# facebookresearch/unbiased-teacher-v2

Measured on AMD Instinct MI355X. Metric: images/sec/node (labeled+unlabeled) UTv2 step, R50-FPN 1333x800, higher is better.
Workload: dtype f16

## Files before the change

include/utv2.h:

```cpp
#ifndef UTV2_H
#define UTV2_H
#include <stdint.h>
#ifdef __cplusplus
extern "C" {
#endif

typedef struct ihipStream_t* utv2_stream_t;

int utv2_conv2d_nhwc_fwd(const float* x, const float* w, float* y, const float* scale, const float* bias,
                         const float* residual, int N, int H, int W, int C, int K, int KH, int KW, int stride, int pad,
                         int in_dil, int OH, int OW, int relu, int accumulate, int Kred, utv2_stream_t stream);
int utv2_conv2d_stem_fwd(const float* x, const float* w, void* y, int y_dtype, const float* scale, const float* bias, int N,
                         int H, int W, int K, int KH, int KW, int stride, int pad, int OH, int OW, int relu, int Kred,
                         utv2_stream_t stream);
int utv2_conv2d_wgrad_splits(int N, int OH, int OW, int K, int Kred);
int64_t utv2_conv2d_wgrad_workspace_floats(int N, int OH, int OW, int K, int Kred);
int utv2_conv2d_nhwc_wgrad(const float* x, const float* dy, float* dw, float* ws, int N, int H, int W, int C, int K,
                           int KH, int KW, int stride, int pad, int OH, int OW, int accumulate, utv2_stream_t stream);
int utv2_colsum(const float* g, float* db, float* ws, int M, int C, int accumulate, utv2_stream_t stream);
int utv2_weight_flip_transpose(const float* w, float* wt, int K, int KH, int KW, int C, utv2_stream_t stream);

int utv2_conv2d_ml_fwd(const float* x, const float* w, float* y, const float* scale, const float* bias,
                       const float* residual, int nlev, const int* H_host, const int* W_host, int N, int C, int K, int KH,
                       int KW, int pad, int relu, int accumulate, utv2_stream_t stream);
// ... 167 lines not shown

int utv2_nms_mpad(int M);
int64_t utv2_nms_workspace_bytes(int N, int M);
int utv2_nms_batched(const float* boxes, const float* scores, const int* cls, const unsigned char* valid, int N, int M,
                     float iou_thr, int class_aware, int post_topk, int max_out, int* keep, int* keep_count, void* ws,
                     utv2_stream_t stream);
int utv2_box_iou(const float* a, const float* b, int A, int B, float* out, utv2_stream_t stream);

int utv2_match_boxes(const float* boxes, int64_t box_img_stride, int N, int P, const float* gt_boxes,
                     const unsigned char* gt_valid, int G, float* max_iou, int* arg, unsigned* gt_max_bits,
                     utv2_stream_t stream);
int utv2_match_lowq(const float* boxes, int64_t box_img_stride, int N, int P, const float* gt_boxes,
                    const unsigned char* gt_valid, int G, const unsigned* gt_max_bits, unsigned char* lowq,
                    utv2_stream_t stream);
int utv2_roi_align_fwd(int num_levels, int min_level, const void* const* feats_host, const int* H_host,
                       const int* W_host, const float* scales_host, const float* rois, const int* roi_batch,
                       const unsigned char* roi_valid, int R, int C, int PH, int PW, void* out, int dtype,
                       utv2_stream_t stream);
int utv2_roi_align_bwd(int num_levels, int min_level, float* const* dfeats_host, const int* H_host, const int* W_host,
                       const float* scales_host, const float* rois, const int* roi_batch, const unsigned char* roi_valid,
                       int R, int C, int PH, int PW, const void* dy, int dtype, utv2_stream_t stream);
int utv2_roi_align_bwd_tiled(int num_levels, int min_level, void* const* dfeats_host, const int* H_host, const int* W_host,
                             const float* scales_host, const float* rois, const unsigned char* roi_valid, int N, int rois_per_image,
                             int C, int PH, int PW, const void* dy, int dy_dtype, int out_dtype, utv2_stream_t stream);
int utv2_rpn_rank_keys(const float* head, int num_levels, const int* hw_host, int N, int A, int ch, int64_t* keys, utv2_stream_t stream);
int utv2_rpn_decode(const int64_t* top, int maxk, const float* head, const float* anchors, const float* image_hw, int num_levels,
                    const int* hw_host, const int* k_host, int N, int A, int ch, const float* weights_host, float scale_clamp,
                    float min_size, float* boxes, float* scores, int* lvls, unsigned char* keep, utv2_stream_t stream);
int utv2_nms_pack(const int* kidx, const int* cnt, const float* boxes, const float* scores, int N, int M, int D, float* oboxes, float* oscores,
                  unsigned char* ovalid, utv2_stream_t stream);
int utv2_roi_infer_keys(const float* probs, const float* deltas, const float* prop, const unsigned char* valid, const float* whwh, int N, int P,
                        int K, float wx, float wy, float scale_clamp, float thr, float* boxes, int64_t* keys, utv2_stream_t stream);
int utv2_roi_infer_gather(const int64_t* top, const float* boxes, int N, int P, int K, int k, float thr, float* sc, int64_t* rows, int* cls,
                          float* cb, unsigned char* valid, utv2_stream_t stream);
int utv2_roi_infer_pack(const int* kidx, const int* cnt, const float* cb, const float* sc, const int* cls, const int64_t* rows, const float* stdl,
                        int N, int P, int k, int D, float* oboxes, float* oscores, int* ocls, float* ostd, int64_t* orows, unsigned char* ovalid,
                        utv2_stream_t stream);
int utv2_rpn_loss_fwd(const float* obj, const float* deltas, int head, int num_levels, const int* hw_host, int N, int A, int ch, int R,
                      const float* anchors, const int64_t* pos_idx, const unsigned char* pos_valid, int npos, const int64_t* neg_idx,
                      const unsigned char* neg_valid, int nneg, const int* matched, const unsigned char* has_gt, const float* gt_boxes,
                      const float* gt_scores, int G, const float* weights_host, float* sums, float* gobj, float* gdl, utv2_stream_t stream);
int utv2_rpn_loss_bwd(const float* gobj, const float* gdl, const float* gout_cls, const float* gout_loc, int head, int num_levels,
                      const int* hw_host, int N, int A, int ch, int R, const int64_t* pos_idx, const unsigned char* pos_valid, int npos,
                      const int64_t* neg_idx, const unsigned char* neg_valid, int nneg, float* grad_obj, float* grad_deltas,
                      utv2_stream_t stream);
int utv2_rpn_loss_fwd_range(const float* obj, const float* deltas, int head, int num_levels, const int* hw_host, int N, int batch, int img0,
                            int A, int ch, int R, const float* anchors, const int64_t* pos_idx, const unsigned char* pos_valid, int npos,
                            const int64_t* neg_idx, const unsigned char* neg_valid, int nneg, const int* matched,
                            const unsigned char* has_gt, const float* gt_boxes, const float* gt_scores, int G, const float* weights_host,
                            float* sums, float* gobj, float* gdl, utv2_stream_t stream);
int utv2_rpn_loss_bwd_range(const float* gobj, const float* gdl, const float* gout_cls, const float* gout_loc, int head, int num_levels,
                            const int* hw_host, int N, int batch, int img0, int A, int ch, int R, const int64_t* pos_idx,
                            const unsigned char* pos_valid, int npos, const int64_t* neg_idx, const unsigned char* neg_valid, int nneg,
                            float* grad_obj, float* grad_deltas, utv2_stream_t stream);
int utv2_rpn_sample_keys(const float* max_iou, const unsigned char* lowq, const unsigned char* gt_valid, int G, const float* keys, int N,
                         int R, float lo, float hi, int64_t* out, utv2_stream_t stream);
int utv2_rpn_sample_unpack(const int64_t* top, int k, int N, int npos_max, int nneg_max, const unsigned char* gt_valid, int G,
                           int64_t* pos_idx, unsigned char* pos_valid, int64_t* neg_idx, unsigned char* neg_valid, unsigned char* has_gt,
                           utv2_stream_t stream);
int utv2_roi_sample(const float* boxes, const unsigned char* valid, const float* max_iou, const int* argmax, const float* keys, int N, int P,
                    const float* gt_boxes, const int* gt_classes, const unsigned char* gt_valid, const float* gt_scores, const float* gt_std,
                    int G, float iou_thr, int num_classes, int batch, int nfg_max, float* out_boxes, int64_t* out_classes,
                    float* out_gt_boxes, unsigned char* out_valid, int64_t* out_idx, float* out_conf, float* out_std, utv2_stream_t stream);
int utv2_roi_box_loss(const float* deltas, const float* stdl, int64_t ld, const int64_t* cls, const float* prop, const float* gtb,
                      const float* gstd, int R, int num_classes, int mode, float wx, float wy, float scale_clamp, float ts_better,
                      float t_cert, float* sum, float* gdeltas, float* gstd_out, utv2_stream_t stream);
int utv2_softmax_focal_fwd(const float* logits, const int* target, int R, int C, float gamma, float* loss_sum, float* ws,
                           utv2_stream_t stream);
int utv2_softmax_focal_bwd(const float* logits, const int* target, int R, int C, float gamma, const float* coef,
                           float* dlogits, utv2_stream_t stream);
int utv2_rcnn_loss_combine(const float* rpn_sup, const float* rpn_uns, const float* focal_sup, const float* focal_uns, const float* box_sup,
                           const float* box_uns, const int* tgt_sup, int n_sup, const int* tgt_uns, int n_uns, float rpn_norm_sup,
                           float rpn_norm_uns, float w_rpn_cls, float w_rpn_loc, float w_box, const float* wt_host, float* rec, float* coef,
                           utv2_stream_t stream);

int utv2_stem_pool_fwd_bf16(const void* xpad16, const void* w16s, void* y, const float* scale, const float* shift, int N, int H, int W,
                            int K, utv2_stream_t stream);

int utv2_bottleneck_supported(int C, int MID, int has_shortcut);
int utv2_bottleneck_fwd_bf16(const void* x, void* y, const void* w1, const void* w2, const void* w3, const void* wsc, const float* s1,
                             const float* b1, const float* s2, const float* b2, const float* s3, const float* b3, const float* ssc,
                             const float* bsc, int N, int H, int W, int C, int MID, utv2_stream_t stream);

int64_t utv2_aug_resize_workspace_bytes(int H, int W, int OH, int OW);
int utv2_aug_resize_bilinear_u8(const unsigned char* src, int H, int W, unsigned char* dst, int OH, int OW, int flip, void* ws,
                                utv2_stream_t stream);
int utv2_aug_gray_mean_u8(const unsigned char* img, int64_t npix, void* sum_ws, int* mean_out, utv2_stream_t stream);
int utv2_aug_blend_u8(unsigned char* img, int64_t npix, int mode, float alpha, const int* mean, utv2_stream_t stream);
int utv2_aug_hue_u8(unsigned char* img, int64_t npix, int shift, utv2_stream_t stream);
int utv2_aug_grayscale_u8(unsigned char* img, int64_t npix, utv2_stream_t stream);
int utv2_aug_box_blur_u8(const unsigned char* src, unsigned char* dst, int H, int W, int vertical, int radius, int ww, int fw,
                         utv2_stream_t stream);
int utv2_aug_erase_u8(unsigned char* img, int H, int W, int i, int j, int h, int w, const float* noise, utv2_stream_t stream);
int utv2_aug_hwc_to_chw_u8(const unsigned char* src, unsigned char* dst, int64_t npix, utv2_stream_t stream);

int utv2_coco_pair_keys(const float* scores, const int* cls, const long long* off, int N, int K, long long* keys, utv2_stream_t stream);
int utv2_coco_seg_offsets(const long long* keys, int64_t n, int64_t nseg, long long* off, utv2_stream_t stream);
int utv2_coco_rank_keys(const long long* key1, const long long* pair_off, int64_t D, int K, int max_dets, long long* key2,
                        unsigned char* rank, utv2_stream_t stream);
int64_t utv2_coco_eval_workspace_bytes(int64_t D, int K);
int utv2_coco_match(const float* dbox, const long long* dperm, const long long* dpair_off, const double* gbox, const unsigned char* gcrowd,
                    const double* garea, const long long* gperm, const long long* gpair_off, int N, int K, int64_t D, int max_dets,
                    int max_gt, const double* iou_thrs_host, const double* area_rng_host, void* ws, utv2_stream_t stream);
int utv2_coco_accumulate(const long long* perm2, const long long* cat_off, const unsigned char* rank, int K, int64_t D,
                         const double* rec_thrs_host, const void* ws, double* precision, double* recall, utv2_stream_t stream);

int utv2_gconv3x3_supported(int C, int G);
int utv2_gconv3x3_fwd(const void* x, const void* w, int op_dtype, void* y, int y_dtype, const float* scale, const float* shift, int N,
                      int H, int W, int C, int G, int stride, int OH, int OW, int relu, utv2_stream_t stream);
int utv2_gconv3x3_dgrad(const void* dy, const void* w, int op_dtype, void* dx, int dx_dtype, const float* scale, const void* mask,
                        const void* residual, int N, int H, int W, int C, int G, int stride, int OH, int OW, utv2_stream_t stream);
int utv2_gconv3x3_wgrad_splits(int N, int OH, int OW, int C, int G);
int64_t utv2_gconv3x3_wgrad_workspace_floats(int N, int OH, int OW, int C, int G);
int utv2_gconv3x3_wgrad(const void* x, const void* dy, int op_dtype, float* dw, float* ws, const float* scale, int N, int H, int W,
                        int C, int G, int stride, int OH, int OW, int accumulate, utv2_stream_t stream);

#ifdef __cplusplus
}
#endif
#endif
```

unbiased-teacher-v2_amd/ubteacher/hip.py:

```python
import ctypes
import os

import torch

_HERE = os.path.dirname(os.path.abspath(__file__))
_LIB_DIR = os.environ.get("UTV2_LIB_DIR") or os.path.join(os.path.dirname(_HERE), "lib")
LIB_PATH = os.path.join(_LIB_DIR, "libutv2_hip.so")
LIB_PATHS = {"bf16": LIB_PATH, "fp16": os.path.join(_LIB_DIR, "libutv2_hip_f16.so")}
H16 = ["bf16"]


_H16_DT = [torch.bfloat16]


def set_h16(kind):
    assert kind in LIB_PATHS
    H16[0] = kind
    _H16_DT[0] = torch.bfloat16 if kind == "bf16" else torch.float16


def h16_dtype():
    return _H16_DT[0]

_lib = None

c_p = ctypes.c_void_p
c_i = ctypes.c_int
c_i64 = ctypes.c_int64
c_f = ctypes.c_float

HEADER_PATH = os.path.join(os.path.dirname(os.path.dirname(_HERE)), "include", "utv2.h")


def _parse_header(path):
    import re

    txt = open(path).read()
    txt = re.sub(r"/\*.*?\*/", "", txt, flags=re.S)
    sigs = {}
    for m in re.finditer(r"\b(int64_t|int)\s+(utv2_\w+)\s*\(([^;{]*?)\)\s*;", txt, flags=re.S):
        ret, name, args = m.group(1), m.group(2), m.group(3)
        argt = []
        for a in [x.strip() for x in args.replace("\n", " ").split(",") if x.strip()]:
            if "*" in a or "utv2_stream_t" in a:
                argt.append(c_p)
            elif a.startswith("int64_t"):
                argt.append(c_i64)
            elif a.startswith("double"):
                argt.append(ctypes.c_double)
            elif a.startswith("float"):
                argt.append(c_f)
            elif a.startswith("int"):
                argt.append(c_i)
            elif a == "void":
                pass
            else:
                raise RuntimeError("utv2.h: cannot map argument %r of %s" % (a, name))
        sigs[name] = (c_i64 if ret == "int64_t" else c_i, argt)
    return sigs


_SIGS = _parse_header(HEADER_PATH)
_PLAIN = {"utv2_aug_resize_workspace_bytes", "utv2_topk_rows_workspace_bytes", "utv2_groupnorm_seg_workspace_floats", "utv2_groupnorm_seg_chunks", "utv2_conv2d_wgrad_bf16_splits", "utv2_conv2d_wgrad_bf16_workspace_floats", "utv2_conv2d_bf16_supported", "utv2_conv2d_wgrad_splits", "utv2_conv2d_wgrad_workspace_floats", "utv2_groupnorm_workspace_floats",
          "utv2_nms_mpad", "utv2_nms_workspace_bytes", "utv2_bottleneck_supported", "utv2_wgrad_fold_table_bytes", "utv2_wgrad_fold_pending",
          "utv2_coco_eval_workspace_bytes", "utv2_gconv3x3_supported", "utv2_gconv3x3_wgrad_splits",
          "utv2_gconv3x3_wgrad_workspace_floats"}


_libs = {}


def load(kind=None):
    kind = kind or H16[0]
    lib = _libs.get(kind)
    if lib is not None:
        return lib
    path = LIB_PATHS[kind]
    if not os.path.exists(path):
        raise RuntimeError(
            "HIP extension %s is missing - run `python __graft_entry__.py` (hipcc, gfx950)" % path
        )
    lib = ctypes.CDLL(path)
    for name, (res, args) in _SIGS.items():
        fn = getattr(lib, name)
        fn.restype = res
        fn.argtypes = args
    _libs[kind] = lib
    return lib


def symbols():
    return sorted(_SIGS)


_RAW_STREAM = getattr(torch._C, "_cuda_getCurrentRawStream", None)
_GET_DEVICE = getattr(torch._C, "_cuda_getDevice", None)


def _stream():
    if _RAW_STREAM is not None and _GET_DEVICE is not None:
        return _RAW_STREAM(_GET_DEVICE())
    return torch.cuda.current_stream().cuda_stream


def _p(t):
    if t is None:
        return None
    assert t.is_cuda and t.is_contiguous(), "HIP ops need contiguous CUDA tensors"
    return t.data_ptr()


def _dt(t):
    d = t.dtype
    if d == torch.float32:
        return 0
    if d == _H16_DT[0]:
        return 1
    raise TypeError("activation tensors are fp32 or %s (the selected library's 16-bit type), got %s" % (h16_dtype(), t.dtype))


def _same_dt(*ts):
    ts = [t for t in ts if t is not None]
    assert all(t.dtype == ts[0].dtype for t in ts), [t.dtype for t in ts]
    return _dt(ts[0])


def _p_any(t):
    return c_p(t.data_ptr())


def _check(rc, name):
    if rc != 0:
        raise RuntimeError("%s failed with code %d" % (name, rc))


_FN = {}


def call(name, *args):
    fn = _FN.get((H16[0], name))
    if fn is None:
        fn = _FN[(H16[0], name)] = getattr(load(), name)
    rc = fn(*args)
    if rc != 0:
        raise RuntimeError("%s failed with code %d" % (name, rc))


# ... 747 lines not shown


def f32_to_bf16(src, dst16):
    call("utv2_f32_to_bf16", _p(src), _p(dst16), src.numel(), _stream())


def weight_flip_transpose_bf16(w, K, kh, kw, C, scale=None):
    wt = torch.empty((C, kh * kw * K), dtype=h16_dtype(), device=w.device)
    call("utv2_weight_flip_transpose_bf16", _p(w), _p(wt), _p(scale), K, kh, kw, C, _stream())
    return wt


def _act_dtype(x, out_dtype):
    return out_dtype if out_dtype is not None else x.dtype


def pad_cols_bf16(src2d, cpad):
    rows, c = src2d.shape
    out = torch.empty((rows, cpad), dtype=h16_dtype(), device=src2d.device)
    call("utv2_pad_cols_bf16", _p(src2d), _dt(src2d), _p(out), rows, c, cpad, _stream())
    return out


def weight_flip_transpose_bf16_batched(arena, scales, bank, table, nlayers):
    call("utv2_weight_flip_transpose_bf16_batched", _p(arena), c_p(scales.data_ptr()) if scales is not None else c_p(0), _p(bank),
         _p(table), int(nlayers), _stream())


def relu_bits_buffer(shape, device):
    assert shape[-1] % 8 == 0
    return torch.empty(tuple(shape[:-1]) + (shape[-1] // 8,), dtype=torch.uint8, device=device)


def _bits_ok(bits, shape):
    n = 1
    for d in shape:
        n *= int(d)
    assert bits.dtype == torch.uint8 and bits.is_contiguous() and bits.numel() * 8 == n, "bit plane of another tensor"
    return bits


def conv2d_fwd_bf16(x, w16, scale=None, bias=None, residual=None, stride=1, pad=0, relu=False, kh=1, kw=1, out=None,
                    in_dil=1, out_hw=None, accumulate=False, out_dtype=None, mask=None, post_mask=None, relu_bits=None):
    N, H, W, C = x.shape
    K = w16.shape[0]
    assert w16.dtype == h16_dtype() and C % 8 == 0
    if out_hw is None:
        OH, OW = conv_out_size(H, kh, stride, pad), conv_out_size(W, kw, stride, pad)
    else:
        OH, OW = out_hw
    if out is None:
        out = torch.empty((N, OH, OW, K), dtype=_act_dtype(x, out_dtype), device=x.device)
    ri = None
    if _CONV_ROWINFO and kh * kw > 1 and in_dil == 1 and x.dtype == h16_dtype() and C % 32 == 0 and kh * kw <= 16 and W < 32768:
        ri = rowinfo_nhwc(N, H, W, OH, OW, stride, pad, kh, kw, x.device)
    if relu_bits is not None:
        assert out.dtype == h16_dtype()
        call("utv2_conv2d_nhwc_fwd_bf16_bits", _p(x), _dt(x), _p(w16), _p(out), _same_dt(out, residual, mask, post_mask), _p(scale), _p(bias),
             _p(residual), _p(mask), _p(post_mask), N, H, W, C, K, kh, kw, stride, pad, in_dil, OH, OW, int(relu), int(accumulate), _p(ri),
             _p(_bits_ok(relu_bits, out.shape)), c_p(0), c_p(0), _stream())
        return out
    call("utv2_conv2d_nhwc_fwd_bf16_ri", _p(x), _dt(x), _p(w16), _p(out), _same_dt(out, residual, mask, post_mask), _p(scale), _p(bias),
         _p(residual), _p(mask), _p(post_mask), N, H, W, C, K, kh, kw, stride, pad, in_dil, OH, OW, int(relu), int(accumulate), _p(ri), _stream())
    return out


def bottleneck_fwd_bf16(x, w1, w2, w3, s1, b1, s2, b2, s3, b3, wsc=None, ssc=None, bsc=None, out=None):
    N, H, W, C = x.shape
    MID, K = w1.shape[0], w3.shape[0]
    assert x.dtype == h16_dtype() and w1.dtype == w2.dtype == w3.dtype == h16_dtype() and K == 256
    assert tuple(w1.shape) == (MID, C) and tuple(w2.shape) == (MID, 9 * MID) and tuple(w3.shape) == (K, MID)
    assert wsc is None or (tuple(wsc.shape) == (K, C) and wsc.dtype == h16_dtype())
    if out is None:
        out = torch.empty((N, H, W, K), dtype=x.dtype, device=x.device)
    call("utv2_bottleneck_fwd_bf16", _p(x), _p(out), _p(w1), _p(w2), _p(w3), _p(wsc), _p(s1), _p(b1), _p(s2), _p(b2), _p(s3), _p(b3),
         _p(ssc), _p(bsc), N, H, W, C, MID, _stream())
    return out


def bottleneck_supported(C, MID, has_shortcut):
    return bool(load().utv2_bottleneck_supported(C, MID, int(has_shortcut)))


def conv2d_dgrad_bf16(dy, wt16, in_shape, stride, pad, kh, kw, out=None, out_dtype=None, mask=None, residual=None, post_mask=None,
                      mask_bits=None, post_mask_bits=None):
    N, H, W, C = in_shape
    _, OH, OW, K = dy.shape
    if out is None:
        out = torch.empty((N, H, W, C), dtype=_act_dtype(dy, out_dtype), device=dy.device)
    ri = None
    if _CONV_ROWINFO and kh * kw > 1 and stride == 1 and dy.dtype == h16_dtype() and K % 32 == 0 and kh * kw <= 16 and OW < 32768:
        ri = rowinfo_nhwc(N, OH, OW, H, W, 1, kh - 1 - pad, kh, kw, dy.device)
    if mask_bits is not None or post_mask_bits is not None:
        assert out.dtype == h16_dtype() and (mask is None or mask_bits is None) and (post_mask is None or post_mask_bits is None)
        call("utv2_conv2d_nhwc_fwd_bf16_bits", _p(dy), _dt(dy), _p(wt16), _p(out), _same_dt(out, residual, mask, post_mask), c_p(0), c_p(0),
             _p(residual), _p(mask), _p(post_mask), N, OH, OW, K, C, kh, kw, 1, kh - 1 - pad, stride, H, W, 0, 0, _p(ri), c_p(0),
             _p(_bits_ok(mask_bits, out.shape)) if mask_bits is not None else c_p(0),
             _p(_bits_ok(post_mask_bits, out.shape)) if post_mask_bits is not None else c_p(0), _stream())
        return out
    call("utv2_conv2d_nhwc_fwd_bf16_ri", _p(dy), _dt(dy), _p(wt16), _p(out), _same_dt(out, residual, mask, post_mask), c_p(0), c_p(0),
         _p(residual), _p(mask), _p(post_mask), N, OH, OW, K, C, kh, kw, 1, kh - 1 - pad, stride, H, W, 0, 0, _p(ri), _stream())
    return out


def _rows_ptr(t):
    assert t.is_cuda and t.dim() == 2 and t.stride(1) == 1 and t.stride(0) >= t.shape[1], "row-major matrix (or a column slice of one) expected"
    return c_p(t.data_ptr()), int(t.stride(0))


def gnb_eligible(x2d, w16, k, pad, groups):
    C = x2d.shape[1] // groups
    K = w16.shape[0]
    return (x2d.dtype == h16_dtype() and C % 64 == 0 and k * k * C >= 1024 and K % groups == 0 and (K // groups) % 128 == 0
            and x2d.stride(1) == 1 and x2d.stride(0) % 8 == 0 and x2d.shape[0] * x2d.stride(0) < (1 << 31))


def gnb_part_buffer(P, K, device):
    return torch.empty(((P + 63) // 64, K, 2), dtype=torch.float32, device=device)


def conv2d_ml_fwd_bf16(x2d, w16, level_hw, N, scale=None, bias=None, residual=None, k=3, pad=1, relu=False, out=None,
                       out_dtype=None, groups=1, gn_part=None, gnb=None):
    P = x2d.shape[0]
    C = x2d.shape[1] // groups
    K = w16.shape[0]
    assert w16.shape[1] == k * k * C, (tuple(w16.shape), k, C)
    if out is None:
        out = torch.empty((P, K), dtype=_act_dtype(x2d, out_dtype), device=x2d.device)
    H = _iarr([h for h, _ in level_hw]); W = _iarr([w_ for _, w_ in level_hw])
    xp, xpitch = _rows_ptr(x2d)
    yp, ypitch = _rows_ptr(out)
    if gnb is not None:
        bits, gx, part = gnb
        assert (scale is None and bias is None and residual is None and not relu and gn_part is None and out.dtype == h16_dtype()
                and ypitch == K and gx.dtype == h16_dtype() and gx.is_contiguous() and tuple(gx.shape) == (P, K)
                and bits.numel() * bits.element_size() * 8 == P * K and tuple(part.shape) == ((P + 63) // 64, K, 2))
        ri = rowinfo_ml(N, level_hw, pad, k, x2d.device) if (_CONV_ROWINFO and k > 1) else None
        call("utv2_conv2d_ml_fwd_bf16_gnb", xp, xpitch, _p(w16), yp, len(level_hw), ctypes.cast(H, c_p), ctypes.cast(W, c_p), N, C, K, k, k,
             pad, int(groups), _p(ri), _p(bits), _p(gx), _p(part), _stream())
        return out
    ri = None
    if (_CONV_ROWINFO and k > 1 and x2d.dtype == h16_dtype() and C % 32 == 0 and K % 4 == 0 and xpitch % 8 == 0 and ypitch % 8 == 0
            and (groups == 1 or (K // groups) % 128 == 0) and P * xpitch < (1 << 31)):
        ri = rowinfo_ml(N, level_hw, pad, k, x2d.device)
    if groups == 1 and xpitch == C and ypitch == K and gn_part is None and ri is None:
        call("utv2_conv2d_ml_fwd_bf16", xp, _dt(x2d), _p(w16), yp, _same_dt(out, residual), _p(scale), _p(bias), _p(residual),
             len(level_hw), ctypes.cast(H, c_p), ctypes.cast(W, c_p), N, C, K, k, k, pad, int(relu), 0, _stream())
    else:
        assert residual is None or (residual.stride(0) == ypitch and residual.stride(1) == 1)
        call("utv2_conv2d_ml_fwd_bf16_g", xp, _dt(x2d), xpitch, _p(w16), yp, _same_dt(out, residual), ypitch, _p(scale), _p(bias),
             c_p(residual.data_ptr()) if residual is not None else c_p(0), len(level_hw), ctypes.cast(H, c_p), ctypes.cast(W, c_p), N, C, K,
             k, k, pad, int(relu), 0, int(groups), _p(gn_part), _p(ri), _stream())
    return out


def gn_part_buffer(P, K, device):
    return torch.empty(((P + 31) // 32, K // 8, 2), dtype=torch.float32, device=device)


def groupnorm_relu_seg_fwd_p32(x2d, seg_rows, gamma, beta, part32, G, eps=1e-5, relu=True, relu_bits=None):
    rows, C = x2d.shape
    assert sum(seg_rows) == rows and x2d.dtype == h16_dtype() and C == 8 * G
    y = torch.empty_like(x2d)
    S = len(seg_rows)
    mean = torch.empty((S, G), dtype=torch.float32, device=x2d.device)
    rstd = torch.empty((S, G), dtype=torch.float32, device=x2d.device)
# ... 346 lines not shown
```

unbiased-teacher-v2_amd/ubteacher/ops.py:

```python
import os

import torch

from . import hip

_HOOKS = {}
PRECISION = ["fp32"]


def set_precision(p):
    assert p in ("fp32", "bf16", "fp16")
    PRECISION[0] = p
    hip.set_h16("fp16" if p == "fp16" else "bf16")


def amp():
    return PRECISION[0] != "fp32"


def act_dtype():
    return hip.h16_dtype() if amp() else torch.float32


_VERSION = [0]
# ... 595 lines not shown
        _wgrad_launch(lambda: hip.gconv3x3_wgrad(x4, g4, layer.w.g, layer.groups, layer.stride, scale=layer.bn.scale, accumulate=True),
                      x4, g4, key=layer)
        return
    n_, h_, w_, _ = x4.shape
    ri = hip.rowinfo_nhwc(n_, h_, w_, g4.shape[1], g4.shape[2], layer.stride, layer.pad, layer.k, layer.k, x4.device)
    _wgrad_launch(lambda: hip.conv2d_wgrad_bf16(x4, g4.reshape(-1, layer.cout), layer.w.g, ri, layer.cin, layer.k, layer.k, accumulate=True,
                                                rowscale=layer.bn.scale), x4, g4, key=layer)


def _dgrad16(layer, g4, in_shape, mask=None, residual=None, post_mask=None, mask_bits=None, post_mask_bits=None):
    if mask_bits is not None:
        mask = None
    if post_mask_bits is not None:
        post_mask = None
    if layer.gconv:
        assert post_mask is None and post_mask_bits is None and mask_bits is None
        return hip.gconv3x3_dgrad(g4, layer.gconv_weight(), layer.groups, layer.stride, tuple(in_shape), scale=layer.bn.scale, mask=mask,
                                  residual=residual, out_dtype=hip.h16_dtype())
    BITS_STATS["reads"] += (mask_bits is not None) + (post_mask_bits is not None)
    return hip.conv2d_dgrad_bf16(g4, layer.wt16(layer.bn.scale), tuple(in_shape), layer.stride, layer.pad, layer.k, layer.k,
                                 out_dtype=hip.h16_dtype(), mask=mask, residual=residual, post_mask=post_mask, mask_bits=mask_bits,
                                 post_mask_bits=post_mask_bits)


class GradHandoff:
    _live = []

    def __init__(self):
        self.grad = None
        self.closed = False
        if len(GradHandoff._live) >= 64:
            del GradHandoff._live[:32]
        GradHandoff._live.append(self)

    def park(self, g):
        if self.closed or self.grad is not None:
            return False
        self.grad = g
        return True

    def take(self):
        self.closed = True
        g, self.grad = self.grad, None
        return g


def grad_handoff_on():
    return premask_on() and os.environ.get("UTV2_GRAD_HANDOFF", "1") != "0"


def relu_bits_on():
    return os.environ.get("UTV2_RELU_BITS", "1") != "0"


BITS_STATS = {"planes": 0, "reads": 0}


def _bits_of(t):
    b = getattr(t, "_utv2_relu_bits", None)
    if b is not None and (b[0] != t.data_ptr() or b[1] != t._version):
        return None
    return None if b is None else b[2]


def premask_on():
    return os.environ.get("UTV2_PREMASK", "1") != "0"


class _BottleneckFn(torch.autograd.Function):
    @staticmethod
    def forward(ctx, x, hk, block):
        c1, c2, c3, cs = block.conv1, block.conv2, block.conv3, block.shortcut
        res = cs._forward(x, None, None, None, None) if cs is not None else x
        b1 = b2 = b3 = None
        if relu_bits_on() and all(c.relu and c.cout % 8 == 0 for c in (c1, c2, c3)):
            planes, (n_, h_, w_, _) = [], x.shape
            for c in (c1, c2, c3):
                h_, w_ = hip.conv_out_size(h_, c.k, c.stride, c.pad), hip.conv_out_size(w_, c.k, c.stride, c.pad)
                planes.append(hip.relu_bits_buffer((n_, h_, w_, c.cout), x.device))
            if c2.gconv:
                planes[0] = planes[1] = None
            b1, b2, b3 = planes
            BITS_STATS["planes"] += sum(b is not None for b in planes)
        y1 = c1._forward(x, None, None, None, None, relu_bits=b1)
        y2 = c2._forward(y1, None, None, None, None, relu_bits=b2)
        y3 = c3._forward(y2, res, None, None, None, relu_bits=b3)
        ctx.block = block
        ctx.handoff = None
        if ctx.needs_input_grad[0] and grad_handoff_on() and getattr(x, "_utv2_handoff", None) is None:
            ctx.handoff = x._utv2_handoff = GradHandoff()
        ctx.bits = (_bits_of(x), b1, b2)
        if b3 is not None:
            y3._utv2_relu_bits = (y3.data_ptr(), y3._version, b3)
        ctx.save_for_backward(x, y1, y2, y3)
        if GRAD_SYNC[0] is not None:
            for l in (c1, c2, c3, cs):
                if l is not None:
                    GRAD_SYNC[0].on_forward(_sync_handles(l))
        return y3

    @staticmethod
    def backward(ctx, dy):
        block = ctx.block
        c1, c2, c3, cs = block.conv1, block.conv2, block.conv3, block.shortcut
        x, y1, y2, y3 = ctx.saved_tensors
        pre = premask_on()
        if pre and block.grad_premasked:
            gm = dy.contiguous()
        else:
            gm = hip.relu_bwd_scale(dy.contiguous(), y3, None)
        pm = x if (pre and block.input_relu) else None
        bx, b1, b2 = ctx.bits
        if pm is None:
            bx = None
        _wgrad16(c3, y2, gm)
        g2 = _dgrad16(c3, gm, y2.shape, mask=y2, mask_bits=b2)
        _wgrad16(c2, y1, g2)
        g1 = _dgrad16(c2, g2, y1.shape, mask=y1, mask_bits=b1)
        _wgrad16(c1, x, g1)
        if cs is not None:
            _wgrad16(cs, x, gm)
        dx = None
        if ctx.needs_input_grad[0]:
            parked = ctx.handoff.take() if ctx.handoff is not None else None
            if parked is not None and (parked.dtype != hip.h16_dtype() or tuple(parked.shape) != tuple(x.shape)):
                raise RuntimeError("GradHandoff: parked gradient of another shape / type")
            if cs is None:
                dx = _dgrad16(c1, g1, x.shape, residual=gm, post_mask=pm, post_mask_bits=bx)
                if parked is not None:
                    dx = dx + parked
            elif c1.stride == 2:
                c = hip.conv2d_fwd_bf16(gm, cs.wt16(cs.bn.scale), out_dtype=hip.h16_dtype())
                c = hip.conv2d_fwd_bf16(g1, c1.wt16(c1.bn.scale), residual=c, out_dtype=hip.h16_dtype())
                dx = hip.zero_interleave2x(c, x.shape[1], x.shape[2], mask=pm if bx is None else None, mask_bits=bx if pm is not None else None,
                                           add=parked)
                BITS_STATS["reads"] += (bx is not None and pm is not None)
            elif cs.stride == 2:
                assert c1.stride == 1 and cs.k == 1 and cs.pad == 0
                c = hip.conv2d_fwd_bf16(gm, cs.wt16(cs.bn.scale), out_dtype=hip.h16_dtype())
                d = hip.zero_interleave2x(c, x.shape[1], x.shape[2], add=parked)
                dx = _dgrad16(c1, g1, x.shape, residual=d, post_mask=pm, post_mask_bits=bx)
            else:
                d = _dgrad16(cs, gm, x.shape, residual=parked)
                dx = _dgrad16(c1, g1, x.shape, residual=d, post_mask=pm, post_mask_bits=bx)
        if GRAD_SYNC[0] is not None:
            for l in (c3, c2, c1, cs):
                if l is not None:
                    GRAD_SYNC[0].on_backward_done(_sync_handles(l))
        return dx, None, None


def _fused_frozen_block_on():
    return os.environ.get("UTV2_FUSED_FROZEN_BLOCK", "1") != "0"


def bottleneck(block, x):
    convs = [c for c in (block.conv1, block.conv2, block.conv3, block.shortcut) if c is not None]
    fused = (amp() and torch.is_grad_enabled() and x.dtype == hip.h16_dtype()
             and all(c.trainable and c.bn is not None and c.bias is None
                     and (c.gconv or (c.use_bf16() and c.use_bf16_wgrad() and c.use_bf16_dgrad())) for c in convs)
             and block.conv1.stride in (1, 2) and block.conv1.k == 1 and block.conv3.k == 1
             and not (block.conv1.gconv or block.conv3.gconv)
             and (block.conv1.stride == 1 or block.conv2.stride == 1)
             and (block.shortcut is None or block.shortcut.stride == max(block.conv1.stride, block.conv2.stride)))
    if fused:
        return _BottleneckFn.apply(x, hook(x.device), block)
    if (amp() and x.dtype == hip.h16_dtype() and x.is_contiguous() and _fused_frozen_block_on()
            and (not torch.is_grad_enabled() or not any(c.trainable for c in convs)) and not x.requires_grad
            and all(c.stride == 1 for c in convs) and block.conv1.k == 1 and block.conv2.k == 3 and block.conv3.k == 1
            and (block.shortcut is None or block.shortcut.k == 1) and block.conv3.cout == 256
            and all(c.bn is not None and c.bias is None and c.use_bf16() for c in convs)
            and x.shape[1] * x.shape[2] * 256 < 2 ** 31
            and block.conv2.groups == 1 and block.conv1.cout <= 64
            and hip.bottleneck_supported(block.conv1.cin, block.conv1.cout, block.shortcut is not None)):
        st = block.conv1.w.store
        (s1, b1), (s2, b2), (s3, b3) = block.conv1.scale_shift(), block.conv2.scale_shift(), block.conv3.scale_shift()
        kw = {}
        if block.shortcut is not None:
            ssc, bsc = block.shortcut.scale_shift()
            kw = dict(wsc=st.bf16(block.shortcut.w), ssc=ssc, bsc=bsc)
        return hip.bottleneck_fwd_bf16(x, st.bf16(block.conv1.w), st.bf16(block.conv2.w), st.bf16(block.conv3.w), s1, b1, s2, b2, s3, b3, **kw)
    sc = block.shortcut(x) if block.shortcut is not None else x
    out = block.conv1(x)
    out = block.conv2(out)
    return block.conv3(out, residual=sc)


class _StemFn(torch.autograd.Function):

    @staticmethod
    def forward(ctx, x4, hk, layer):
        sc, sh = layer.scale_shift()
        y = hip.conv2d_stem_fwd(x4, layer.w.t, sc, sh, layer.stride, layer.pad, layer.k, layer.k, True, act_dtype())
        ctx.layer = layer
        ctx.save_for_backward(x4, y)
        if GRAD_SYNC[0] is not None:
            GRAD_SYNC[0].on_forward(_sync_handles(layer))
        return hip.maxpool3x3s2(y)

    @staticmethod
    def backward(ctx, dpool):
        layer = ctx.layer
        x4, y = ctx.saved_tensors
        g = hip.maxpool3x3s2_bwd(y, dpool.contiguous(), relu=True)
        g = g.float() * layer.bn.scale
        K, kred = layer.cout, layer.k * layer.k * layer.cin

        def wgrad():
            dw = torch.empty((K, kred), dtype=torch.float32, device=g.device)
            hip.conv2d_wgrad(x4, g, dw, layer.stride, layer.pad, layer.k, layer.k, accumulate=False)
            layer.w.g.view(K, -1)[:, :kred] += dw
        _wgrad_launch(wgrad, x4, g, key=layer)
        if GRAD_SYNC[0] is not None:
            GRAD_SYNC[0].on_backward_done(_sync_handles(layer))
        return None, None, None


def stem(layer, x4):
    return _StemFn.apply(x4, hook(x4.device), layer)


class ColPair:

    def __init__(self):
        self.buf = None

    def grad_half(self, idx, x):
        if self.buf is None:
            self.buf = torch.empty((x.shape[0], 2 * x.shape[1]), dtype=x.dtype, device=x.device)
        C = x.shape[1]
        return self.buf[:, idx * C:(idx + 1) * C]

    def take(self, g0, g1):
        b, self.buf = self.buf, None
        if (b is not None and g0 is not None and g1 is not None and g0.dtype == b.dtype and g0.data_ptr() == b.data_ptr()
                and g1.data_ptr() == b.data_ptr() + g0.shape[1] * b.element_size() and g0.stride(0) == b.stride(0) == g1.stride(0)):
            return b
        return None


class _SplitColsFn(torch.autograd.Function):
    @staticmethod
    def forward(ctx, t, pair):
        C = t.shape[1] // 2
        ctx.pair, ctx.C = pair, C
        ctx.meta_ = (t.dtype, t.device, t.shape[0])
        return t[:, :C], t[:, C:]

    @staticmethod
    def backward(ctx, g0, g1):
        b = ctx.pair.take(g0, g1)
        if b is not None:
            return b, None
        dt, dev, P = ctx.meta_
        z = None
        if g0 is None or g1 is None:
            z = torch.zeros((P, ctx.C), dtype=dt, device=dev)
        return torch.cat((g0 if g0 is not None else z, g1 if g1 is not None else z), dim=1), None


def split_cols(t):
    C = t.shape[1] // 2
    if not (torch.is_grad_enabled() and t.requires_grad):
        return t[:, :C], t[:, C:]
# ... 394 lines not shown
```

Baseline: 342.1.

## Fuse res3 bottleneck 1x1-3x3-1x1 convs into a single HIP kernel

Adds a fused kernel for the non-shortcut 512→128→512 res3 bottleneck blocks. It keeps conv1 output with halo and conv2 output in LDS, then applies BN, ReLU and the residual add in place, while still writing the c1/c2 activations and ReLU sign bits needed for backward during training. The goal is to remove two intermediate global round-trips and the extra kernel launches. The cost is halo recomputation and heavy LDS use, which may limit occupancy. The no-grad path is off by default.

```diff
diff --git a/include/utv2.h b/include/utv2.h
--- a/include/utv2.h
+++ b/include/utv2.h
@@ -273,6 +273,11 @@
                              const float* b1, const float* s2, const float* b2, const float* s3, const float* b3, const float* ssc,
                              const float* bsc, int N, int H, int W, int C, int MID, utv2_stream_t stream);
 
+int utv2_bottleneck_res3_supported(int C, int MID, int COUT);
+int utv2_bottleneck_res3_fwd_bf16(const void* x, void* y, const void* w1, const void* w2, const void* w3, const float* s1, const float* b1,
+                                  const float* s2, const float* b2, const float* s3, const float* b3, void* c1, void* c2, void* bits1,
+                                  void* bits2, void* bits3, int N, int H, int W, int C, int MID, int COUT, utv2_stream_t stream);
+
 int64_t utv2_aug_resize_workspace_bytes(int H, int W, int OH, int OW);
 int utv2_aug_resize_bilinear_u8(const unsigned char* src, int H, int W, unsigned char* dst, int OH, int OW, int flip, void* ws,
                                 utv2_stream_t stream);
diff --git a/unbiased-teacher-v2_amd/csrc/bottleneck_res3.hip b/unbiased-teacher-v2_amd/csrc/bottleneck_res3.hip
--- /dev/null
+++ b/unbiased-teacher-v2_amd/csrc/bottleneck_res3.hip
@@ -0,0 +1,414 @@
+#include "common.h"
+
+#define B3_TH 8
+#define B3_TW 16
+#define B3_HW 18
+#define B3_HALO 180
+#define B3_HP 192
+#define B3_CIN 512
+#define B3_MID 128
+#define B3_COUT 512
+#define B3_R0 32768
+#define B3_R1 (B3_HALO * 256)
+#define B3_LDS (B3_R0 + B3_R1 + 512 * 4)
+#define B3_XCHUNK (B3_HP * 64)
+
+struct Bt3Args {
+  const h16_t* x;
+  h16_t* y;
+  const h16_t *w1, *w2, *w3;
+  const float *s1, *b1, *s2, *b2, *s3, *b3;
+  h16_t *c1, *c2;
+  unsigned char *bits1, *bits2, *bits3;
+  int N, H, W, tiles_x, tiles_y, ntiles;
+  int o64;
+};
+
+__device__ __forceinline__ bf16x8_t b3_frag(const unsigned char* smem, int off) { return *(const bf16x8_t*)(smem + off); }
+
+__device__ __forceinline__ void b3_piece(int i, int o64, int& tap, int& ch0) {
+  if (o64) {
+    const int h = i / 18, r = i % 18;
+    tap = r >> 1;
+    ch0 = h * 64 + (r & 1) * 32;
+  } else {
+    tap = i % 9;
+    ch0 = (i / 9) * 32;
+  }
+}
+
+__device__ __forceinline__ unsigned b3_signs(bf16x8_t v) {
+  unsigned b = 0;
+#pragma unroll
+  for (int q = 0; q < 8; ++q) b |= ((float)v[q] > 0.f ? 1u : 0u) << q;
+  return b;
+}
+
+template <bool TRAIN>
+__global__ __launch_bounds__(256, 2) void bottleneck_res3_fused(Bt3Args a) {
+  constexpr int NCH = B3_CIN / 32;
+  extern __shared__ __attribute__((aligned(16))) unsigned char smem[];
+  unsigned char* stageA = smem;
+  unsigned char* stageB = smem + B3_R0;
+  unsigned char* c1 = smem + B3_R0;
+  unsigned char* c2 = smem;
+  unsigned char* w3l = smem + B3_R0;
+  float* prm = (float*)(smem + B3_R0 + B3_R1);
+  const int tid = threadIdx.x, lane = tid & 63, wave = tid >> 6, l31 = lane & 31, fh = lane >> 5;
+
+  int t;
+  {
+    const int bid = blockIdx.x, q = a.ntiles >> 3, r = a.ntiles & 7, xcd = bid & 7, idx = bid >> 3;
+    t = (xcd < r ? xcd * (q + 1) : r * (q + 1) + (xcd - r) * q) + idx;
+  }
+  const int per = a.tiles_x * a.tiles_y;
+  const int n = t / per, rem = t - n * per, ty = rem / a.tiles_x, tx = rem - ty * a.tiles_x;
+  const int y0 = ty * B3_TH, x0 = tx * B3_TW;
+  const h16_t* ximg = a.x + (size_t)n * a.H * a.W * B3_CIN;
+
+  const h16_t* xsrc[3];
+  int xdst[3];
+#pragma unroll
+  for (int i = 0; i < 3; ++i) {
+    const int q = tid + 256 * i, px = q >> 2, slot = q & 3;
+    const int hy = px / B3_HW, hx = px - hy * B3_HW, gy = y0 - 1 + hy, gx = x0 - 1 + hx;
+    const bool ok = px < B3_HALO && gy >= 0 && gy < a.H && gx >= 0 && gx < a.W;
+    xsrc[i] = ok ? ximg + ((size_t)gy * a.W + gx) * B3_CIN + slot * 8 : nullptr;
+    xdst[i] = px * 64 + ((slot ^ ((px >> 2) & 3)) << 4);
+  }
+  const h16_t* wsrc[2];
+  int wdst[2];
+#pragma unroll
+  for (int i = 0; i < 2; ++i) {
+    const int q = tid + 256 * i, co = q >> 2, slot = q & 3;
+    wsrc[i] = a.w1 + co * B3_CIN + slot * 8;
+    wdst[i] = B3_XCHUNK + co * 64 + ((slot ^ ((co >> 2) & 3)) << 4);
+  }
+
+  bf16x8_t xr[3][3], wr[3][2];
+  const bf16x8_t zero8 = {};
+#pragma unroll
+  for (int c = 0; c < 3; ++c) {
+#pragma unroll
+    for (int i = 0; i < 3; ++i) xr[c][i] = xsrc[i] ? *(const bf16x8_t*)(xsrc[i] + c * 32) : zero8;
+#pragma unroll
+    for (int i = 0; i < 2; ++i) wr[c][i] = *(const bf16x8_t*)(wsrc[i] + c * 32);
+  }
+  prm[tid] = tid < 128 ? a.s1[tid] : a.b1[tid - 128];
+  prm[256 + tid] = tid < 128 ? a.s2[tid] : a.b2[tid - 128];
+#pragma unroll
+  for (int i = 0; i < 3; ++i) *(bf16x8_t*)(stageA + xdst[i]) = xr[0][i];
+#pragma unroll
+  for (int i = 0; i < 2; ++i) *(bf16x8_t*)(stageA + wdst[i]) = wr[0][i];
+  __syncthreads();
+
+  f32x16 acc1[3][2];
+#pragma unroll
+  for (int i = 0; i < 3; ++i)
+#pragma unroll
+    for (int j = 0; j < 2; ++j)
+#pragma unroll
+      for (int e = 0; e < 16; ++e) acc1[i][j][e] = 0.f;
+  const int pg1 = wave >> 1, cg = wave & 1;
+  const int t2co[2] = {tid >> 2, (tid + 256) >> 2}, t2slot = tid & 3;
+  bf16x8_t tr[3][2][2];
+  auto load_step = [&](int st, bf16x8_t (&dst)[2][2]) {
+#pragma unroll
+    for (int u = 0; u < 2; ++u) {
+      int tap, ch0;
+      b3_piece(2 * st + u, a.o64, tap, ch0);
+#pragma unroll
+      for (int i = 0; i < 2; ++i) dst[u][i] = *(const bf16x8_t*)(a.w2 + t2co[i] * (9 * B3_MID) + tap * B3_MID + ch0 + t2slot * 8);
+    }
+  };
+  auto store_step = [&](unsigned char* buf, const bf16x8_t (&src)[2][2]) {
+#pragma unroll
+    for (int u = 0; u < 2; ++u)
+#pragma unroll
+      for (int i = 0; i < 2; ++i) *(bf16x8_t*)(buf + u * 8192 + t2co[i] * 64 + ((t2slot ^ ((t2co[i] >> 2) & 3)) << 4)) = src[u][i];
+  };
+#pragma unroll
+  for (int kc = 0; kc < NCH; ++kc) {
+    unsigned char* cur = (kc & 1) ? stageB : stageA;
+    unsigned char* nxt = (kc & 1) ? stageA : stageB;
+    if (kc + 3 < NCH) {
+#pragma unroll
+      for (int i = 0; i < 3; ++i) xr[kc % 3][i] = xsrc[i] ? *(const bf16x8_t*)(xsrc[i] + (kc + 3) * 32) : zero8;
+#pragma unroll
+      for (int i = 0; i < 2; ++i) wr[kc % 3][i] = *(const bf16x8_t*)(wsrc[i] + (kc + 3) * 32);
+    } else {
+      load_step(kc - (NCH - 3), tr[kc - (NCH - 3)]);
+    }
+#pragma unroll
+    for (int ks = 0; ks < 2; ++ks) {
+      const int slot = ks * 2 + fh;
+      bf16x8_t xa[3], wa[2];
+#pragma unroll
+      for (int i = 0; i < 3; ++i) {
+        const int row = (3 * pg1 + i) * 32 + l31;
+        xa[i] = b3_frag(cur, row * 64 + ((slot ^ ((row >> 2) & 3)) << 4));
+      }
+#pragma unroll
+      for (int j = 0; j < 2; ++j) {
+        const int row = (2 * cg + j) * 32 + l31;
+        wa[j] = b3_frag(cur, B3_XCHUNK + row * 64 + ((slot ^ ((row >> 2) & 3)) << 4));
+      }
+#pragma unroll
+      for (int i = 0; i < 3; ++i)
+#pragma unroll
+        for (int j = 0; j < 2; ++j) acc1[i][j] = mfma_32x32x16(wa[j], xa[i], acc1[i][j]);
+    }
+    if (kc + 1 < NCH) {
+#pragma unroll
+      for (int i = 0; i < 3; ++i) *(bf16x8_t*)(nxt + xdst[i]) = xr[(kc + 1) % 3][i];
+#pragma unroll
+      for (int i = 0; i < 2; ++i) *(bf16x8_t*)(nxt + wdst[i]) = wr[(kc + 1) % 3][i];
+    }
+    __syncthreads();
+  }
+
+#pragma unroll
+  for (int i = 0; i < 3; ++i) {
+    const int px = (3 * pg1 + i) * 32 + l31;
+    const int hy = px / B3_HW, hx = px - hy * B3_HW, gy = y0 - 1 + hy, gx = x0 - 1 + hx;
+    const bool ok = gy >= 0 && gy < a.H && gx >= 0 && gx < a.W;
+    if (px < B3_HALO) {
+#pragma unroll
+      for (int j = 0; j < 2; ++j)
+#pragma unroll
+        for (int q = 0; q < 4; ++q) {
+          const int ch = (2 * cg + j) * 32 + 8 * q + 4 * fh;
+          const f32x4 sc = *(const f32x4*)(prm + ch), bi = *(const f32x4*)(prm + 128 + ch);
+          bf16x4_t o;
+#pragma unroll
+          for (int e = 0; e < 4; ++e) {
+            float v = acc1[i][j][4 * q + e] * sc[e] + bi[e];
+            v = ok ? fmaxf(v, 0.f) : 0.f;
+            o[e] = (h16_t)v;
+          }
+          *(bf16x4_t*)(c1 + px * 256 + (((ch >> 3) ^ (px & 15)) << 4) + fh * 8) = o;
+        }
+    }
+  }
+  store_step(stageA, tr[0]);
+  __syncthreads();
+
+  const int cpc = tid >> 4, cps = tid & 15;
+  const bool cpx = x0 + cpc < a.W;
+  const size_t cpo = (((size_t)n * a.H + y0) * a.W + x0 + cpc) * B3_MID + cps * 8;
+  if constexpr (TRAIN) {
+#pragma unroll
+    for (int i = 0; i < 8; ++i) {
+      const int h = (i + 1) * B3_HW + cpc + 1;
+      const bf16x8_t v = b3_frag(c1, h * 256 + ((cps ^ (h & 15)) << 4));
+      if (cpx && y0 + i < a.H) {
+        const size_t o = cpo + (size_t)i * a.W * B3_MID;
+        *(bf16x8_t*)(a.c1 + o) = v;
+        a.bits1[o >> 3] = (unsigned char)b3_signs(v);
+      }
+    }
+  }
+
+  f32x16 acc2[2][2];
+#pragma unroll
+  for (int i = 0; i < 2; ++i)
+#pragma unroll
+    for (int j = 0; j < 2; ++j)
+#pragma unroll
+      for (int e = 0; e < 16; ++e) acc2[i][j][e] = 0.f;
+  const int pg2 = wave >> 1;
+  int hb[2];
+#pragma unroll
+  for (int i = 0; i < 2; ++i) {
+    const int p = (2 * pg2 + i) * 32 + l31;
+    hb[i] = (p >> 4) * B3_HW + (p & 15);
+  }
+  const int qslot = tid & 15;
+  bf16x8_t wq[4];
+  auto load_w3 = [&](int g) {
+#pragma unroll
+    for (int i = 0; i < 4; ++i) wq[i] = *(const bf16x8_t*)(a.w3 + (g * 64 + ((tid + 256 * i) >> 4)) * B3_MID + qslot * 8);
+  };
+  auto store_w3 = [&](int g) {
+#pragma unroll
+    for (int i = 0; i < 4; ++i) {
+      const int co = (tid + 256 * i) >> 4;
+      *(bf16x8_t*)(w3l + (g & 1) * 16384 + co * 256 + ((qslot ^ (co & 15)) << 4)) = wq[i];
+    }
+  };
+#pragma unroll
+  for (int st = 0; st < 18; ++st) {
+    unsigned char* cur = stageA + (st & 1) * 16384;
+    unsigned char* nxt = stageA + ((st + 1) & 1) * 16384;
+    if (st + 3 < 18) load_step(st + 3, tr[st % 3]);
+    else if (st == 15) load_w3(0);
+#pragma unroll
+    for (int u = 0; u < 2; ++u) {
+      int tap, ch0;
+      b3_piece(2 * st + u, a.o64, tap, ch0);
+      const int dy = tap / 3, dx = tap - dy * 3, hoff = dy * B3_HW + dx;
+#pragma unroll
+      for (int ks = 0; ks < 2; ++ks) {
+        const int cslot = (ch0 >> 3) + ks * 2 + fh, wslot = ks * 2 + fh;
+        bf16x8_t xf[2], wf[2];
+#pragma unroll
+        for (int i = 0; i < 2; ++i) {
+          const int h = hb[i] + hoff;
+          xf[i] = b3_frag(c1, h * 256 + ((cslot ^ (h & 15)) << 4));
+        }
+#pragma unroll
+        for (int j = 0; j < 2; ++j) {
+          const int row = (2 * cg + j) * 32 + l31;
+          wf[j] = b3_frag(cur, u * 8192 + row * 64 + ((wslot ^ ((row >> 2) & 3)) << 4));
+        }
+#pragma unroll
+        for (int i = 0; i < 2; ++i)
+#pragma unroll
+          for (int j = 0; j < 2; ++j) acc2[i][j] = mfma_32x32x16(wf[j], xf[i], acc2[i][j]);
+      }
+    }
+    if (st + 1 < 18) store_step(nxt, tr[(st + 1) % 3]);
+    __syncthreads();
+  }
+  const int sub = lane >> 3, cv = lane & 7;
+  int opix[4];
+#pragma unroll
+  for (int i = 0; i < 4; ++i) {
+    const int pp = wave * 32 + 8 * i + sub, gy = y0 + (pp >> 4), gx = x0 + (pp & 15);
+    opix[i] = (gy < a.H && gx < a.W) ? ((gy * a.W + gx) * B3_COUT + cv * 8) : -1;
+  }
+  h16_t* yout = a.y + (size_t)n * a.H * a.W * B3_COUT;
+  unsigned char* ybits = TRAIN ? a.bits3 + (size_t)n * a.H * a.W * (B3_COUT / 8) : nullptr;
+  bf16x8_t res[2][4];
+#pragma unroll
+  for (int i = 0; i < 4; ++i) res[0][i] = opix[i] >= 0 ? *(const bf16x8_t*)(ximg + opix[i]) : zero8;
+#pragma unroll
+  for (int i = 0; i < 2; ++i) {
+    const int p = (2 * pg2 + i) * 32 + l31;
+#pragma unroll
+    for (int j = 0; j < 2; ++j)
+#pragma unroll
+      for (int q = 0; q < 4; ++q) {
+        const int ch = (2 * cg + j) * 32 + 8 * q + 4 * fh;
+        const f32x4 sc = *(const f32x4*)(prm + 256 + ch), bi = *(const f32x4*)(prm + 384 + ch);
+        bf16x4_t o;
+#pragma unroll
+        for (int e = 0; e < 4; ++e) o[e] = (h16_t)fmaxf(acc2[i][j][4 * q + e] * sc[e] + bi[e], 0.f);
+        *(bf16x4_t*)(c2 + p * 256 + (((ch >> 3) ^ (p & 15)) << 4) + fh * 8) = o;
+      }
+  }
+  store_w3(0);
+  __syncthreads();
+  load_w3(1);
+
+  const int p3 = wave * 32 + l31;
+  bf16x8_t cf[8];
+#pragma unroll
+  for (int ks = 0; ks < 8; ++ks) cf[ks] = b3_frag(c2, p3 * 256 + (((ks * 2 + fh) ^ (p3 & 15)) << 4));
+  if constexpr (TRAIN) {
+#pragma unroll
+    for (int i = 0; i < 8; ++i) {
+      const int p = i * 16 + cpc;
+      const bf16x8_t v = b3_frag(c2, p * 256 + ((cps ^ (p & 15)) << 4));
+      if (cpx && y0 + i < a.H) {
+        const size_t o = cpo + (size_t)i * a.W * B3_MID;
+        *(bf16x8_t*)(a.c2 + o) = v;
+        a.bits2[o >> 3] = (unsigned char)b3_signs(v);
+      }
+    }
+  }
+  __syncthreads();
+  float* patch = (float*)smem + wave * (16 * 64);
+#pragma unroll
+  for (int g = 0; g < 8; ++g) {
+    if (g + 1 < 8) {
+      store_w3(g + 1);
+      if (g + 2 < 8) load_w3(g + 2);
+#pragma unroll
+      for (int i = 0; i < 4; ++i) res[(g + 1) & 1][i] = opix[i] >= 0 ? *(const bf16x8_t*)(ximg + opix[i] + (g + 1) * 64) : zero8;
+    }
+    f32x16 acc3[2];
+#pragma unroll
+    for (int u = 0; u < 2; ++u)
+#pragma unroll
+      for (int e = 0; e < 16; ++e) acc3[u][e] = 0.f;
+    const unsigned char* wb = w3l + (g & 1) * 16384;
+#pragma unroll
+    for (int ks = 0; ks < 8; ++ks) {
+#pragma unroll
+      for (int u = 0; u < 2; ++u) {
+        const int row = u * 32 + l31;
+        const bf16x8_t wf = b3_frag(wb, row * 256 + (((ks * 2 + fh) ^ (row & 15)) << 4));
+        acc3[u] = mfma_32x32x16(wf, cf[ks], acc3[u]);
+      }
+    }
+    const f32x4 s3a = *(const f32x4*)(a.s3 + g * 64 + cv * 8), s3b = *(const f32x4*)(a.s3 + g * 64 + cv * 8 + 4);
+    const f32x4 b3a = *(const f32x4*)(a.b3 + g * 64 + cv * 8), b3b = *(const f32x4*)(a.b3 + g * 64 + cv * 8 + 4);
+#pragma unroll
+    for (int hh = 0; hh < 2; ++hh) {
+      if ((l31 >> 4) == hh) {
+        const int prow = l31 & 15;
+#pragma unroll
+        for (int u = 0; u < 2; ++u)
+#pragma unroll
+          for (int q = 0; q < 4; ++q) {
+            const int cl = u * 32 + 8 * q + 4 * fh;
+            const f32x4 v = {acc3[u][4 * q], acc3[u][4 * q + 1], acc3[u][4 * q + 2], acc3[u][4 * q + 3]};
+            *(f32x4*)(patch + prow * 64 + (((cl >> 2) ^ prow) << 2)) = v;
+          }
+      }
+      __builtin_amdgcn_s_waitcnt(0xc07f);
+      __builtin_amdgcn_wave_barrier();
+#pragma unroll
+      for (int i2 = 0; i2 < 2; ++i2) {
+        const int i = hh * 2 + i2, prow = 8 * i2 + sub;
+        const f32x4 v0 = *(const f32x4*)(patch + prow * 64 + (((2 * cv) ^ prow) << 2)), v1 = *(const f32x4*)(patch + prow * 64 + (((2 * cv + 1) ^ prow) << 2));
+        bf16x8_t o;
+#pragma unroll
+        for (int j = 0; j < 4; ++j) {
+          o[j] = (h16_t)fmaxf(v0[j] * s3a[j] + b3a[j] + (float)res[g & 1][i][j], 0.f);
+          o[4 + j] = (h16_t)fmaxf(v1[j] * s3b[j] + b3b[j] + (float)res[g & 1][i][4 + j], 0.f);
+        }
+        if (opix[i] >= 0) {
+          *(bf16x8_t*)(yout + opix[i] + g * 64) = o;
+          if constexpr (TRAIN) ybits[(opix[i] + g * 64) >> 3] = (unsigned char)b3_signs(o);
+        }
+      }
+      __builtin_amdgcn_s_waitcnt(0xc07f);
+      __builtin_amdgcn_wave_barrier();
+    }
+    if (g + 1 < 8) __syncthreads();
+  }
+}
+
+extern "C" {
+
+int utv2_bottleneck_res3_supported(int C, int MID, int COUT) { return C == B3_CIN && MID == B3_MID && COUT == B3_COUT; }
+
+int utv2_bottleneck_res3_fwd_bf16(const void* x, void* y, const void* w1, const void* w2, const void* w3, const float* s1, const float* b1,
+                                  const float* s2, const float* b2, const float* s3, const float* b3, void* c1, void* c2, void* bits1,
+                                  void* bits2, void* bits3, int N, int H, int W, int C, int MID, int COUT, hipStream_t stream) {
+  if (!x || !y || x == y || !w1 || !w2 || !w3 || !s1 || !b1 || !s2 || !b2 || !s3 || !b3 || N < 1 || H < 1 || W < 1) return UTV2_EARG;
+  if (!utv2_bottleneck_res3_supported(C, MID, COUT)) return UTV2_EARG;
+  const bool train = c1 != nullptr;
+  if (train ? (!c2 || !bits1 || !bits2 || !bits3) : (c2 || bits1 || bits2 || bits3)) return UTV2_EARG;
+  if ((long long)H * W * B3_COUT > 0x7fffffffll || (long long)N * H * W > 0x7fffffffll) return UTV2_EARG;
+  Bt3Args a;
+  a.x = (const h16_t*)x; a.y = (h16_t*)y; a.w1 = (const h16_t*)w1; a.w2 = (const h16_t*)w2; a.w3 = (const h16_t*)w3;
+  a.s1 = s1; a.b1 = b1; a.s2 = s2; a.b2 = b2; a.s3 = s3; a.b3 = b3;
+  a.c1 = (h16_t*)c1; a.c2 = (h16_t*)c2; a.bits1 = (unsigned char*)bits1; a.bits2 = (unsigned char*)bits2; a.bits3 = (unsigned char*)bits3;
+  a.N = N; a.H = H; a.W = W;
+  a.tiles_x = cdiv(W, B3_TW); a.tiles_y = cdiv(H, B3_TH);
+  const long long nt = (long long)N * a.tiles_x * a.tiles_y;
+  if (nt > 0x7fffffff) return UTV2_EARG;
+  a.ntiles = (int)nt;
+  const int ctiles = cdiv(N * H * W, 128);
+  a.o64 = !(ctiles > 512 && ctiles <= 768);
+  static LdsOptIn lds_opt_in;
+  lds_opt_in({(const void*)bottleneck_res3_fused<false>, (const void*)bottleneck_res3_fused<true>}, B3_LDS);
+  if (train) hipLaunchKernelGGL((bottleneck_res3_fused<true>), dim3((unsigned)a.ntiles), dim3(256), B3_LDS, stream, a);
+  else hipLaunchKernelGGL((bottleneck_res3_fused<false>), dim3((unsigned)a.ntiles), dim3(256), B3_LDS, stream, a);
+  return utv2_launch_status();
+}
+
+}
diff --git a/unbiased-teacher-v2_amd/ubteacher/hip.py b/unbiased-teacher-v2_amd/ubteacher/hip.py
--- a/unbiased-teacher-v2_amd/ubteacher/hip.py
+++ b/unbiased-teacher-v2_amd/ubteacher/hip.py
@@ -62,7 +62,7 @@
 
 _SIGS = _parse_header(HEADER_PATH)
 _PLAIN = {"utv2_aug_resize_workspace_bytes", "utv2_topk_rows_workspace_bytes", "utv2_groupnorm_seg_workspace_floats", "utv2_groupnorm_seg_chunks", "utv2_conv2d_wgrad_bf16_splits", "utv2_conv2d_wgrad_bf16_workspace_floats", "utv2_conv2d_bf16_supported", "utv2_conv2d_wgrad_splits", "utv2_conv2d_wgrad_workspace_floats", "utv2_groupnorm_workspace_floats",
-          "utv2_nms_mpad", "utv2_nms_workspace_bytes", "utv2_bottleneck_supported", "utv2_wgrad_fold_table_bytes", "utv2_wgrad_fold_pending",
+          "utv2_nms_mpad", "utv2_nms_workspace_bytes", "utv2_bottleneck_supported", "utv2_bottleneck_res3_supported", "utv2_wgrad_fold_table_bytes", "utv2_wgrad_fold_pending",
           "utv2_coco_eval_workspace_bytes", "utv2_gconv3x3_supported", "utv2_gconv3x3_wgrad_splits",
           "utv2_gconv3x3_wgrad_workspace_floats"}
 
@@ -976,6 +976,30 @@
     return bool(load().utv2_bottleneck_supported(C, MID, int(has_shortcut)))
 
 
+def bottleneck_res3_fwd_bf16(x, w1, w2, w3, s1, b1, s2, b2, s3, b3, keep=None, out=None):
+    N, H, W, C = x.shape
+    MID, K = w1.shape[0], w3.shape[0]
+    assert x.dtype == h16_dtype() and w1.dtype == w2.dtype == w3.dtype == h16_dtype()
+    assert tuple(w1.shape) == (MID, C) and tuple(w2.shape) == (MID, 9 * MID) and tuple(w3.shape) == (K, MID)
+    if out is None:
+        out = torch.empty((N, H, W, K), dtype=x.dtype, device=x.device)
+    if keep is None:
+        call("utv2_bottleneck_res3_fwd_bf16", _p(x), _p(out), _p(w1), _p(w2), _p(w3), _p(s1), _p(b1), _p(s2), _p(b2), _p(s3), _p(b3),
+             None, None, None, None, None, N, H, W, C, MID, K, _stream())
+        return out
+    c1 = torch.empty((N, H, W, MID), dtype=x.dtype, device=x.device)
+    c2 = torch.empty_like(c1)
+    bits1, bits2, bits3 = keep
+    call("utv2_bottleneck_res3_fwd_bf16", _p(x), _p(out), _p(w1), _p(w2), _p(w3), _p(s1), _p(b1), _p(s2), _p(b2), _p(s3), _p(b3),
+         _p(c1), _p(c2), _p(_bits_ok(bits1, c1.shape)), _p(_bits_ok(bits2, c2.shape)), _p(_bits_ok(bits3, out.shape)), N, H, W, C, MID, K,
+         _stream())
+    return out, c1, c2
+
+
+def bottleneck_res3_supported(C, MID, COUT):
+    return bool(load().utv2_bottleneck_res3_supported(C, MID, COUT))
+
+
 def conv2d_dgrad_bf16(dy, wt16, in_shape, stride, pad, kh, kw, out=None, out_dtype=None, mask=None, residual=None, post_mask=None,
                       mask_bits=None, post_mask_bits=None):
     N, H, W, C = in_shape
diff --git a/unbiased-teacher-v2_amd/ubteacher/ops.py b/unbiased-teacher-v2_amd/ubteacher/ops.py
--- a/unbiased-teacher-v2_amd/ubteacher/ops.py
+++ b/unbiased-teacher-v2_amd/ubteacher/ops.py
@@ -701,9 +701,13 @@
                 planes[0] = planes[1] = None
             b1, b2, b3 = planes
             BITS_STATS["planes"] += sum(b is not None for b in planes)
-        y1 = c1._forward(x, None, None, None, None, relu_bits=b1)
-        y2 = c2._forward(y1, None, None, None, None, relu_bits=b2)
-        y3 = c3._forward(y2, res, None, None, None, relu_bits=b3)
+        if b1 is not None and b2 is not None and b3 is not None and res3_block_eligible(block, x):
+            RES3_STATS["train"] += 1
+            y3, y1, y2 = hip.bottleneck_res3_fwd_bf16(x, *_res3_operands(block), keep=(b1, b2, b3))
+        else:
+            y1 = c1._forward(x, None, None, None, None, relu_bits=b1)
+            y2 = c2._forward(y1, None, None, None, None, relu_bits=b2)
+            y3 = c3._forward(y2, res, None, None, None, relu_bits=b3)
         ctx.block = block
         ctx.handoff = None
         if ctx.needs_input_grad[0] and grad_handoff_on() and getattr(x, "_utv2_handoff", None) is None:
@@ -769,6 +773,32 @@
         return dx, None, None
 
 
+def fused_res3_on(nograd=False):
+    if os.environ.get("UTV2_FUSED_RES3", "1") == "0":
+        return False
+    return not nograd or os.environ.get("UTV2_FUSED_RES3_NOGRAD", "0") == "1"
+
+
+RES3_STATS = {"train": 0, "nograd": 0}
+
+
+def res3_block_eligible(block, x, nograd=False):
+    c1, c2, c3 = block.conv1, block.conv2, block.conv3
+    return (fused_res3_on(nograd) and amp() and block.shortcut is None and x.dtype == hip.h16_dtype() and x.is_contiguous() and x.dim() == 4
+            and all(c.stride == 1 and c.groups == 1 and not c.gconv and c.bn is not None and c.bias is None and c.relu and c.use_bf16()
+                    for c in (c1, c2, c3))
+            and c1.k == 1 and c1.pad == 0 and c2.k == 3 and c2.pad == 1 and c3.k == 1 and c3.pad == 0
+            and x.shape[3] == c1.cin and c1.cout == c2.cin == c2.cout == c3.cin and c3.cout == c1.cin
+            and x.shape[1] * x.shape[2] * c3.cout < 2 ** 31 and x.shape[0] * x.shape[1] * x.shape[2] < 2 ** 31
+            and hip.bottleneck_res3_supported(c1.cin, c1.cout, c3.cout))
+
+
+def _res3_operands(block):
+    st = block.conv1.w.store
+    (s1, b1), (s2, b2), (s3, b3) = block.conv1.scale_shift(), block.conv2.scale_shift(), block.conv3.scale_shift()
+    return st.bf16(block.conv1.w), st.bf16(block.conv2.w), st.bf16(block.conv3.w), s1, b1, s2, b2, s3, b3
+
+
 def _fused_frozen_block_on():
     return os.environ.get("UTV2_FUSED_FROZEN_BLOCK", "1") != "0"
 
@@ -799,6 +829,9 @@
             ssc, bsc = block.shortcut.scale_shift()
             kw = dict(wsc=st.bf16(block.shortcut.w), ssc=ssc, bsc=bsc)
         return hip.bottleneck_fwd_bf16(x, st.bf16(block.conv1.w), st.bf16(block.conv2.w), st.bf16(block.conv3.w), s1, b1, s2, b2, s3, b3, **kw)
+    if ((not torch.is_grad_enabled() or not (x.requires_grad or any(c.trainable for c in convs))) and res3_block_eligible(block, x, nograd=True)):
+        RES3_STATS["nograd"] += 1
+        return hip.bottleneck_res3_fwd_bf16(x, *_res3_operands(block))
     sc = block.shortcut(x) if block.shortcut is not None else x
     out = block.conv1(x)
     out = block.conv2(out)
```

Result: no change. 342.1, median of 2 (+0.0%).
